# octree-nn/octfusion

Measured on AMD Instinct MI355X. Metric: denoising-steps/sec (depth-8 octree, batch 8), higher is better.
Workload: dtype f32 storage, fp16x3 products (fp16 hi + lo operand pairs = 22 significand bits, three fp16 MFMAs per product, fp32 accumulate)

## Files before the change

### include/ofx.h

```cpp
#ifndef OFX_H_
#define OFX_H_

#include <stddef.h>
#include <stdint.h>

#ifdef __cplusplus
extern "C" {
#endif

#define OFX_OK 0
#define OFX_EINVAL (-1)
#define OFX_ELAUNCH (-2)
#define OFX_ENODEV (-3)

#define OFX_ACT_NONE 0
#define OFX_ACT_SILU 1
#define OFX_ACT_GELU 2

#define OFX_MAX_DEPTH 16

int ofx_version(void);
const char* ofx_status_string(int status);
int ofx_device_check(void);
const char* ofx_build_hash(void);
// ... 140 lines not shown
int ofx_get_precision(void);
int64_t ofx_packed_floats(int64_t Kp, int64_t N);
int64_t ofx_packed_k(int64_t K);
int64_t ofx_graphconv_packed_k(int cin, int nt);
int ofx_pack_weights(const float* W, int64_t sk, int64_t sn, int64_t K, int64_t N,
                     int cin, int nt, float* Wp, int64_t Kp, void* stream);

int ofx_gemm_f32(const float* A, int64_t lda, const int32_t* a_rows, int64_t M, int64_t K,
                 const float* Wp, int64_t Kp, int64_t N, const float* bias,
                 const float* res, int64_t ldr, float* out, int64_t ldc,
                 const int32_t* out_rows, void* ws, size_t ws_bytes, void* stream);
int ofx_gemm_f32_planes(const float* A, int64_t lda, const int32_t* a_rows, int64_t M, int64_t K,
                        const float* Wp, int64_t Kp, int64_t N, const float* bias,
                        const float* res, int64_t ldr, float* out, int64_t ldc,
                        const int32_t* out_rows, void* ws, size_t ws_bytes, int out_mode, void* stream);

int ofx_graphconv_fwd(const float* x, int64_t ldx, int cin, int64_t n_nodes,
                      const int32_t* nbr, const int32_t* seg_ptr, const int32_t* col,
                      const int32_t* nbr_ext, const int32_t* multi_seg, int64_t n_multi, float* aux,
                      const float* type_frac, int64_t ldt, int nt_pad,
                      const float* Wp, int64_t Kp, int cout, const float* bias,
                      const float* emb, int64_t lde, const int32_t* batch_id,
                      const float* res, int64_t ldr, float* out, int64_t ldc,
                      double* stats , int64_t stats_ld,
                      void* ws, size_t ws_bytes, void* stream);

int ofx_graphconv_narrow_in(const float* x, int64_t ldx, int cin, int64_t n_nodes, const int32_t* seg_ptr,
                            const int32_t* col, const uint8_t* node_type, int nt, const float* W, int cout,
                            const float* bias, const int32_t* batch_id, float* out, int64_t ldc,
                            double* stats , int64_t stats_ld, void* ws, size_t ws_bytes, void* stream);
// ... 47 lines not shown
int ofx_graphconv_fwd_planes(const void* xp, int64_t ldx_bytes, int cin, int64_t n_nodes, const int32_t* seg_ptr,
                             const int32_t* col, const int32_t* nbr_ext, const int32_t* multi_seg, int64_t n_multi,
                             void* aux, size_t aux_bytes, const void* tfp, int64_t ldt_bytes, int nt, const void* W2,
                             int cout, const float* bias, const float* emb, int64_t lde, const int32_t* batch_id,
                             const float* res, int64_t ldr, float* out, int64_t ldc, double* stats ,
                             int64_t stats_ld, void* ws, size_t ws_bytes, void* sync , size_t sync_bytes,
                             int mode, int aux_ready, void* stream);
int ofx_graphconv_fwd_planes_cus(const void* xp, int64_t ldx_bytes, int cin, int64_t n_nodes, const int32_t* seg_ptr,
                                 const int32_t* col, const int32_t* nbr_ext, const int32_t* multi_seg, int64_t n_multi,
                                 void* aux, size_t aux_bytes, const void* tfp, int64_t ldt_bytes, int nt,
                                 const void* W2, int cout, const float* bias, const float* emb, int64_t lde,
                                 const int32_t* batch_id, const float* res, int64_t ldr, float* out, int64_t ldc,
                                 double* stats , int64_t stats_ld, void* ws, size_t ws_bytes,
                                 void* sync , size_t sync_bytes, int mode, int aux_ready, int cus,
                                 void* stream);
int ofx_set_gconv_persistent(int on);
int64_t ofx_gemm_planes_packed_bytes(int K, int N, int mode);
int ofx_pack_gemm_planes(const float* W, int64_t sk, int64_t sn, int K, int N, int mode, void* out, void* stream);
int ofx_gemm_planes(const void* ap, int64_t lda_bytes, int64_t n_a, int64_t M, int K, const int32_t* row_tab,
                    const void* W2, int N, const float* bias, float* out, int64_t ldc, int out_mode, void* ws,
                    size_t ws_bytes, void* sync, size_t sync_bytes, int mode, void* stream);
int ofx_set_gconv_cus(int cus);
int ofx_gconv3_plan(int64_t n_rows, int cout, int nkt, int wm, int ni, int cus, int32_t* out, int64_t out_len);
int ofx_set_gconv2_tile(int wm);

int ofx_grid_conv_table(int mode, int depth_out, int batch_size, int32_t pad, int32_t* nbr27,
                        void* stream);
int64_t ofx_conv3d_packed_k(int cin);
int ofx_pack_conv3d(const float* W, int cin, int cout, float* Wp, void* stream);
int ofx_gridconv_fwd(const float* x, int64_t ldx, int cin, int64_t n_in, int64_t n_out,
                     const int32_t* nbr27 ,
                     const int32_t* nbr27_ext ,
                     const float* zero_row ,
                     const float* Wp, int cout, const float* bias, const float* emb, int64_t lde,
                     const int32_t* batch_id, const float* res, int64_t ldr, float* out,
                     int64_t ldc, void* ws, size_t ws_bytes, void* stream);
int ofx_gather_gemm_f32(const float* x, int64_t ldx, int cin, int ntap, int64_t n_src, int64_t n_out, const int32_t* tab,
                        const float* zero_row, const float* Wp, int64_t Kp, int cout, const float* bias,
// ... 188 lines not shown
```

### octfusion_amd/_lib.py

```python
import ctypes
import os

import torch

_HERE = os.path.dirname(os.path.abspath(__file__))
LIB_PATH = os.environ.get('OFX_LIB', os.path.join(_HERE, 'libofx.so'))

c_p = ctypes.c_void_p
c_i = ctypes.c_int
c_l = ctypes.c_int64
c_f = ctypes.c_float
c_d = ctypes.c_double
c_sz = ctypes.c_size_t
c_u64 = ctypes.c_uint64


class OfxTree(ctypes.Structure):
    _fields_ = [('depth', c_i), ('full_depth', c_i), ('batch_size', c_i),
                ('child_all', c_p), ('key_all', c_p), ('leafrank_all', c_p),
                ('nnum_host', c_p), ('nnum_nempty_host', c_p)]


class OfxAdamRow(ctypes.Structure):
    _fields_ = [('param', c_p), ('grad', c_p), ('exp_avg', c_p), ('exp_avg_sq', c_p), ('ema', c_p), ('n', c_l)]
# ... 89 lines not shown
    'ofx_planes_split': (c_i, [c_p, c_l, c_l, c_i, c_i, c_i, c_p, c_l, c_p], True),
    'ofx_planes_merge': (c_i, [c_p, c_l, c_l, c_i, c_i, c_p, c_l, c_p], True),
    'ofx_gn_apply_planes': (c_i, [c_p, c_l, c_l, c_i, c_p, c_p, c_p, c_p, c_p, c_i, c_f, c_f, c_p, c_p, c_i, c_i, c_p,
                                  c_l, c_p, c_p, c_p, c_l, c_p, c_p, c_l, c_p], True),
    'ofx_gn_apply_planes_oct': (c_i, [c_p, c_l, c_l, c_i, c_p, c_p, c_p, c_p, c_p, c_i, c_f, c_f, c_p, c_p, c_i, c_i, c_p,
                                      c_l, c_l, c_p, c_p, c_p, c_l, c_i, c_p, c_p, c_l, c_p], True),
    'ofx_planes_packed_ktiles': (c_l, [c_i, c_i, c_i], False),
    'ofx_planes_packed_bytes': (c_l, [c_i, c_i, c_i, c_i], False),
    'ofx_pack_weights_planes': (c_i, [c_p, c_l, c_l, c_i, c_i, c_i, c_i, c_p, c_p], True),
    'ofx_graphconv_fwd_planes': (c_i, [c_p, c_l, c_i, c_l, c_p, c_p, c_p, c_p, c_l, c_p, c_sz, c_p, c_l, c_i, c_p, c_i,
                                       c_p, c_p, c_l, c_p, c_p, c_l, c_p, c_l, c_p, c_l, c_p, c_sz, c_p, c_sz, c_i, c_i,
                                       c_p], True),
    'ofx_graphconv_fwd_planes_cus': (c_i, [c_p, c_l, c_i, c_l, c_p, c_p, c_p, c_p, c_l, c_p, c_sz, c_p, c_l, c_i, c_p,
                                           c_i, c_p, c_p, c_l, c_p, c_p, c_l, c_p, c_l, c_p, c_l, c_p, c_sz, c_p, c_sz,
                                           c_i, c_i, c_i, c_p], True),
    'ofx_gn_finalize_window': (c_i, [c_p, c_p, c_i, c_i, c_i, c_i, c_i, c_f, c_f, c_p, c_p, c_p], True),
    'ofx_gn_apply_planes_window': (c_i, [c_p, c_l, c_l, c_i, c_i, c_i, c_p, c_p, c_p, c_p, c_p, c_i, c_f, c_f, c_p, c_p,
                                         c_i, c_i, c_p, c_l, c_p, c_p, c_p, c_l, c_p, c_p, c_l, c_p], True),
    'ofx_gn_apply_planes_oct_window': (c_i, [c_p, c_l, c_l, c_i, c_i, c_i, c_p, c_p, c_p, c_p, c_p, c_i, c_f, c_f, c_p,
                                             c_p, c_i, c_i, c_p, c_l, c_l, c_p, c_p, c_p, c_l, c_i, c_p, c_p, c_l, c_p],
                                       True),
    'ofx_set_gconv_persistent': (c_i, [c_i], True),
    'ofx_set_gconv_cus': (c_i, [c_i], True),
    'ofx_gemm_planes_packed_bytes': (c_l, [c_i, c_i, c_i], False),
    'ofx_pack_gemm_planes': (c_i, [c_p, c_l, c_l, c_i, c_i, c_i, c_p, c_p], True),
    'ofx_gemm_planes': (c_i, [c_p, c_l, c_l, c_l, c_i, c_p, c_p, c_i, c_p, c_p, c_l, c_i, c_p, c_sz, c_p, c_sz, c_i, c_p], False),
    'ofx_gconv3_plan': (c_i, [c_l, c_i, c_i, c_i, c_i, c_i, c_p, c_l], False),
    'ofx_set_gconv2_tile': (c_i, [c_i], True),
    'ofx_graph_multi_flag': (c_i, [c_p, c_l, c_p, c_p], True),
    'ofx_graph_primary_ext': (c_i, [c_p, c_p, c_l, c_p, c_p, c_p, c_p], True),
# ... 192 lines not shown
```

### octfusion_amd/csrc/ofx_gemm.hip

```cpp
#include "ofx_gemm_common.h"

constexpr int BM = 128;
constexpr int BK = 32;
constexpr int A_LD = BK + 4;
constexpr int MODE_DENSE = 0;
constexpr int MODE_GATHER = 1;

struct TileCoords { int split, tm, tn; };
__device__ __forceinline__ TileCoords tile_coords(const GemmArgs& g) {
  const int ntile = g.ntm * g.ntn;
  int bid = ofx_xcd_swizzle(blockIdx.x, ntile * g.nsplit);
  const int split = bid / ntile;
  bid -= split * ntile;
  const int tm = bid / g.ntn;
  return {split, tm, bid - tm * g.ntn};
}

__device__ __forceinline__ void load_a_dense(const GemmArgs& g, int64_t m0, int64_t k0, float4 (&va)[4]) {
  const int c4 = threadIdx.x & 7, r0 = threadIdx.x >> 3;
  const int64_t k = k0 + c4 * 4;
  const bool vec = ((g.lda & 3) == 0) && (k + 3 < g.K) && ((((uintptr_t)g.A) & 15) == 0);
#pragma unroll
  for (int i = 0; i < 4; ++i) {
    const int64_t m = m0 + r0 + 32 * i;
// ... 794 lines not shown
      }
      s += (double)v[i].x; q += (double)v[i].y;
    }
    if (sb >= 0) flush(sb, s, q);
  }
}

int ofx_launch_stats_reduce(const GemmArgs& g, int wr_rows, hipStream_t st) {
  const int64_t nwr = ofx_cdiv(g.M, wr_rows);
  stats_reduce_kernel<<<dim3((unsigned)ofx_cdiv(nwr, 64), (unsigned)ofx_cdiv(g.N, 64)), 256, 0, st>>>(
      g.stats_part, nwr, wr_rows, g.N, g.bid, g.stats, g.stats_ld);
  OFX_LAUNCH_CHECK();
  return OFX_OK;
}

template <int MODE>
static int launch_gemm(GemmArgs& g, float* ws, size_t ws_bytes, hipStream_t st) {
  if (g.M <= 0 || g.N <= 0) return OFX_OK;
  if (MODE == MODE_GATHER && !(g.fast && g.nbr_ext && g.aux && (!g.out_rows || g.gather_out_rows))) return OFX_EINVAL;
  {
    auto al16 = [](const void* p) { return (reinterpret_cast<uintptr_t>(p) & 15) == 0; };
    g.vec4 = g.N % 4 == 0 && al16(g.out) && g.ldc % 4 == 0 && (!g.res || (al16(g.res) && g.ldr % 4 == 0)) &&
             (!g.emb || (al16(g.emb) && g.lde % 4 == 0)) && (!g.bias || al16(g.bias));
  }
  const int bn = g.N <= 32 ? 32 : (g.N <= 64 ? 64 : 128);
  g.ntm = (int)ofx_cdiv(g.M, BM);
  g.ntn = (int)ofx_cdiv(g.N, bn);
  const int nkt = (int)(g.Kp / BK);
  int nsplit = 1;
  const int tiles = g.ntm * g.ntn;
  if (ws && tiles < 256 && nkt >= 8) {
    nsplit = (int)ofx_cdiv(512, tiles);
    if (nsplit > nkt / 4) nsplit = nkt / 4;
    if (nsplit > 64) nsplit = 64;
    const size_t per = (size_t)g.M * g.N * sizeof(float);
    if ((size_t)nsplit * per > ws_bytes) nsplit = (int)(ws_bytes / per);
    if (nsplit < 2) nsplit = 1;
  }
  g.kt_per_split = (int)ofx_cdiv(nkt, nsplit);
  nsplit = (int)ofx_cdiv(nkt, g.kt_per_split);
  g.nsplit = nsplit;
  g.ws = ws;
  bool fast = true;
  if (MODE == MODE_DENSE) {
    fast = ((g.lda & 3) == 0) && ((g.K & 3) == 0) && g.K >= 4 && ((((uintptr_t)g.A) & 15) == 0);
    if (fast) { g.ndir = 1; g.n_src = 0; g.aux = g.A; g.tf = g.A; g.ldt = g.lda; g.nbr_ext = (const int32_t*)g.A; }
  }
// ... 696 lines not shown
```

### octfusion_amd/csrc/ofx_gemm2.hip

```cpp
#include "ofx_planes.h"

template <int PREC, int WM, int NI>
__global__ void __launch_bounds__(512, 2) gconv2_kernel(const Gemm2Args a) {
  typedef G2Half<PREC, NI> Half;
  typedef G2Cfg<WM, NI> CF;
  constexpr int G2_NI = NI, G2_BN = CF::BN, G2_EPI_LOADS = CF::EPI_LOADS, RH = CF::READS;
  constexpr int G2_WM = WM, G2_BM = CF::BM, G2_A_BYTES = CF::A_BYTES, G2_BUF = CF::BUF, G2_TAB = CF::TAB;
  constexpr int G2_GLDS_PER_STEP = CF::GLDS;
  extern __shared__ __attribute__((aligned(128))) char smem2[];
  const GemmArgs& g = a.e;

  float osc = *g.oscale_p;
  asm volatile("" : "+s"(osc));
  const int ntile = g.ntm * g.ntn;
  const int bid = ofx_xcd_swizzle(blockIdx.x, ntile);
  const int tm = bid / g.ntn, tn = bid - tm * g.ntn;
  const int64_t m0 = a.row0 + (int64_t)tm * G2_BM, n0 = (int64_t)tn * G2_BN;

  const int lane = threadIdx.x & 63;
  const int wid = __builtin_amdgcn_readfirstlane(threadIdx.x >> 6);
  const int wm = wid >> 1, wn = wid & 1;
  const int l31 = lane & 31, h = lane >> 5;
  if (WM == 2 && a.stagger > 0 && blockIdx.x >= 256 && (int)blockIdx.x < a.prefetch) {
    const int grp = (int)blockIdx.x >> 8, ngrp = a.prefetch >> 8;
// ... 532 lines not shown
constexpr int G2_STAGGER_PER_KTILE = 1100;
extern "C" int ofx_set_gconv2_tile(int wm) {
  if (wm != 0 && wm != 2 && wm != 4) return OFX_EINVAL;
  g2_wm = wm;
  return OFX_OK;
}

static int g3_wm_pref = 0;
static int g3_auto_wm(int64_t M, int cout, int nkt, int ni) {
  (void)cout; (void)ni;
  if (g3_wm_pref == 2 || g3_wm_pref == 4) return g3_wm_pref;
  const int64_t U4 = ofx_cdiv(M, 256) * ofx_cdiv(cout, 64 * ni) * nkt;
  return U4 >= 3500 ? 4 : 2;
}
int ofx_launch_gconv3(Gemm2Args& a, int mode, int wm, int ni, void* ws_tail, size_t ws_tail_bytes, void* sync,
                      size_t sync_bytes, hipStream_t st, int nd = 7, int cus = 0);
static int g2_persistent = 1;
void ofx_gconv3_set_hybrid(int on);
extern "C" int ofx_set_gconv_persistent(int on) {
  if (on < 0 || on > 2) return OFX_EINVAL;
  g2_persistent = on ? 1 : 0;
  ofx_gconv3_set_hybrid(on == 2 ? 0 : 1);
  return OFX_OK;
}

extern "C" int ofx_graphconv_fwd_planes_cus(const void* xp, int64_t ldx_bytes, int cin, int64_t n_nodes,
                                            const int32_t* seg_ptr, const int32_t* col, const int32_t* nbr_ext,
                                            const int32_t* multi_seg, int64_t n_multi, void* aux, size_t aux_bytes,
                                            const void* tfp, int64_t ldt_bytes, int nt, const void* W2, int cout,
                                            const float* bias, const float* emb, int64_t lde, const int32_t* batch_id,
                                            const float* res, int64_t ldr, float* out, int64_t ldc, double* stats,
                                            int64_t stats_ld, void* ws, size_t ws_bytes, void* sync, size_t sync_bytes,
                                            int mode, int aux_ready, int cus, void* stream) {
  if (mode < 1 || mode > 3 || cus < 0 || (cus > 0 && cus < 8)) return OFX_EINVAL;
  const int64_t ch = g2_chunk(mode);
  if (n_nodes == 0 && cin >= 1 && cout >= 1) return OFX_OK;
  if (n_nodes < 0 || cin < 1 || (cin % ch) || cout < 1 || !xp || !seg_ptr || !col || !nbr_ext || !aux || !W2 || !out ||
      ldx_bytes < (int64_t)cin * (g2_pairs(mode) ? 4 : 2) || (ldx_bytes & 127) || ((uintptr_t)xp & 127) ||
      ((uintptr_t)aux & 127) || ((uintptr_t)W2 & 127) || ldc < cout || (res && ldr < cout) ||
      (emb && (!batch_id || lde < cout)) || n_multi < 0 || (n_multi > 0 && !multi_seg) || nt < 0)
    return OFX_EINVAL;
  if (aux_bytes < (size_t)(n_multi + 1) * (size_t)ldx_bytes) return OFX_EINVAL;
  const int ntc = nt > 1 ? nt : 0;
  if (ntc > 0 && (!tfp || (ldt_bytes & 127) || ((uintptr_t)tfp & 127) ||
                  ldt_bytes < (7 * (int64_t)ntc + ch - 1) / ch * G2_LINE))
    return OFX_EINVAL;
  if (stats && (!batch_id || stats_ld < cout)) return OFX_EINVAL;
  hipStream_t st = ofx_stream(stream);
  if (!aux_ready)
// ... 30 lines not shown
    a.row0 = row0;
    g.ntm = (int)ofx_cdiv(rows, wm * 64);
    a.stagger = wm == 2 ? G2_STAGGER_PER_KTILE * a.nkt : 0;
    a.prefetch = wm == 4 ? 256 : (ni == 1 ? 768 : 512);
    return mode == 2 ? G2_GO(2, wm) : (mode == 3 ? G2_GO(3, wm) : G2_GO(1, wm));
  };
  const int64_t tiles4 = ofx_cdiv(g.M, 256) * g.ntn;
  const int64_t tail4 = tiles4 % 256;
  const bool small_tail = tail4 > 0 && tail4 <= 64 && tiles4 < 1536;
  int wm_auto = (cout <= 128 && tiles4 < 2048) ? 2 : 4;
  if (cout > 128 && small_tail) wm_auto = 2;
  rc = 1;
  if (g2_persistent && sync) {
    size_t used = 0;
    if (g.stats_part) used = ((size_t)ofx_cdiv(g.M, 64) * (size_t)g.N * 2 * sizeof(float) + 255) & ~(size_t)255;
    const int wm3 = (g2_wm == 2 || g2_wm == 4) ? g2_wm : g3_auto_wm(g.M, cout, a.nkt, ni);
    if (ws && used <= ws_bytes)
      rc = ofx_launch_gconv3(a, mode, wm3, ni, (char*)ws + used, ws_bytes - used, sync, sync_bytes, st, 7, cus);
    if (rc < 0) return rc;
  }
  if (rc == 1) rc = launch((g2_wm == 2 || g2_wm == 4) ? g2_wm : wm_auto, 0, g.M);
#undef G2_GO
  if (rc) return rc;
  if (g.stats_part) {
    rc = ofx_launch_stats_reduce(g, 64, st);
    if (rc) return rc;
  }
  OFX_LAUNCH_CHECK();
  return OFX_OK;
}

extern "C" int ofx_graphconv_fwd_planes(const void* xp, int64_t ldx_bytes, int cin, int64_t n_nodes,
                                        const int32_t* seg_ptr, const int32_t* col, const int32_t* nbr_ext,
                                        const int32_t* multi_seg, int64_t n_multi, void* aux, size_t aux_bytes,
                                        const void* tfp, int64_t ldt_bytes, int nt, const void* W2, int cout,
                                        const float* bias, const float* emb, int64_t lde, const int32_t* batch_id,
                                        const float* res, int64_t ldr, float* out, int64_t ldc, double* stats,
                                        int64_t stats_ld, void* ws, size_t ws_bytes, void* sync, size_t sync_bytes,
                                        int mode, int aux_ready, void* stream) {
  return ofx_graphconv_fwd_planes_cus(xp, ldx_bytes, cin, n_nodes, seg_ptr, col, nbr_ext, multi_seg, n_multi, aux,
                                      aux_bytes, tfp, ldt_bytes, nt, W2, cout, bias, emb, lde, batch_id, res, ldr, out,
                                      ldc, stats, stats_ld, ws, ws_bytes, sync, sync_bytes, mode, aux_ready, 0, stream);
}

// ... 27 lines not shown
```

### octfusion_amd/csrc/ofx_gemm3.hip

```cpp
#include "ofx_planes.h"

constexpr int G3_NSP = 5;
constexpr int G3_KMIN = G3_NSP + 3;

template <int WM, int NI> struct G3Cfg : G2Cfg<WM, NI> {
  typedef G2Cfg<WM, NI> B;
  static constexpr int TAB = B::NBUF * B::BUF;
  static constexpr int RAW = TAB + B::BM * 32;
  static constexpr int RAW_WAVE = 32 * 28;
  static constexpr int LDS = RAW + B::BM * 28 + 128;
};

struct Gemm3Args {
  Gemm2Args b;
  int G;
  unsigned q, rem;
  unsigned U;
  int dp_rounds;
  float* part;
  unsigned* flags;
  unsigned* err;
  const char* nbr_lim;
  int snap;
  int early;
// ... 601 lines not shown
  if (hipGetDevice(&dev) != hipSuccess || dev < 0 || dev >= OFX_MAX_DEVICES) return 0;
  if (!cus[dev]) {
    int n = 0;
    if (hipDeviceGetAttribute(&n, hipDeviceAttributeMultiprocessorCount, dev) != hipSuccess) return 0;
    cus[dev] = n;
  }
  return cus[dev];
}
static int g3_cus() {
  const int n = g3_device_cus();
  return g3_cus_override > 0 && g3_cus_override < n ? g3_cus_override : n;
}

struct G3Plan { int G; unsigned q, rem, U; int dp_rounds; size_t part_bytes; };
static int g3_hybrid = 1;
static bool g3_plan(int64_t M, int cout, int nkt, int wm, int ni, G3Plan& p, int cus = 0) {
  if (cus <= 0) cus = g3_cus();
  if (cus < 8 || nkt < G3_KMIN) return false;
  const int64_t tiles = ofx_cdiv(M, wm * 64) * ofx_cdiv(cout, 64 * ni);
  if (tiles * nkt >= (1ll << 31)) return false;
  int64_t slots = ((int64_t)cus * (wm == 4 ? 1 : 2)) & ~7ll;
  int64_t G, region_tiles;
  int rounds = 0;
  if (tiles >= slots) {
    G = slots;
    rounds = g3_hybrid ? (int)(tiles / G - 1) : 0;
    region_tiles = tiles - (int64_t)rounds * G;
  } else {
    const int64_t U = tiles * nkt;
    G = slots < U / (2 * G3_KMIN) ? slots : U / (2 * G3_KMIN);
    G &= ~7ll;
    region_tiles = tiles;
  }
  if (G < 8) return false;
  const int64_t U = region_tiles * nkt;
  p.G = (int)G; p.U = (unsigned)U; p.q = (unsigned)(U / G); p.rem = (unsigned)(U % G); p.dp_rounds = rounds;
  p.part_bytes = (size_t)G * (size_t)(wm * 64) * (size_t)(64 * ni) * sizeof(float);
  return true;
}

void ofx_gconv3_set_hybrid(int on) { g3_hybrid = on ? 1 : 0; }
extern "C" int ofx_set_gconv_cus(int cus) {
  if (cus < 0 || (cus > 0 && cus < 8)) return OFX_EINVAL;
  g3_cus_override = cus;
  return OFX_OK;
}

extern "C" int ofx_gconv3_plan(int64_t n_rows, int cout, int nkt, int wm, int ni, int cus, int32_t* out, int64_t out_len) {
  G3Plan p;
  if (n_rows <= 0 || cout <= 0 || nkt <= 0 || (wm != 2 && wm != 4) || (ni != 1 && ni != 2)) return 0;
  if (!g3_plan(n_rows, cout, nkt, wm, ni, p, cus)) return 0;
  if (out) {
    if (out_len < 5 + (int64_t)p.G + 1) return 0;
    out[0] = p.G; out[1] = (int32_t)p.q; out[2] = (int32_t)p.rem; out[3] = (int32_t)p.U; out[4] = p.dp_rounds;
    for (int b = 0; b <= p.G; ++b) out[5 + b] = (int32_t)g3_bound((unsigned)b, p.q, p.rem, (unsigned)nkt, true);
  }
  return p.G;
}

int ofx_launch_gconv3(Gemm2Args& a, int mode, int wm, int ni, void* ws_tail, size_t ws_tail_bytes, void* sync,
                      size_t sync_bytes, hipStream_t st, int nd, int cus) {
  G3Plan p;
  GemmArgs& g = a.e;
  if (cus > 0) {
    const int dev_cus = g3_device_cus();
    if (dev_cus <= 0) return 1;
    if (cus > dev_cus) cus = dev_cus;
  }
  if (!sync || ((uintptr_t)sync & 3) || !ws_tail || ((uintptr_t)ws_tail & 15)) return 1;
  if (!g.vec4) return 1;
  if (!g3_plan(g.M, (int)g.N, a.nkt, wm, ni, p, cus)) return 1;
  if (p.part_bytes > ws_tail_bytes || (size_t)(p.G + 1) * sizeof(unsigned) > sync_bytes) return 1;
  if ((a.ldx >> 7) >= (1 << 20) || (a.ldt >> 7) >= (1 << 20) || a.n_src >= (1ll << 31)) return 1;
  Gemm3Args A = {};
  a.row0 = 0;
  g.ntm = (int)ofx_cdiv(g.M, wm * 64);
  A.b = a;
  A.G = p.G; A.q = p.q; A.rem = p.rem; A.U = p.U; A.dp_rounds = p.dp_rounds;
  A.part = (float*)ws_tail; A.flags = (unsigned*)sync;
  A.err = (unsigned*)sync + (sync_bytes / sizeof(unsigned) - 1);
  A.snap = 1;
  A.xcd_contig = 0;
  A.rt = p.U / (unsigned)a.nkt;
  A.early = p.q >= (unsigned)a.nkt ? 1 : 0;
  A.nbr_lim = (const char*)a.nbr_ext + ((((size_t)g.M * 28 - 4) >> 4) << 4);
  if (((uintptr_t)a.nbr_ext & 15)) return 1;
// ... 14 lines not shown
```

### octfusion_amd/graph_unet_hr.py

```python
import inspect

import torch
import torch.nn as nn

from . import ops
from .modules import (GraphConv, GraphDownsample, GraphResBlockEmbed, GraphUpsample, _Linear,
                      graphnormalization, skip_window)


def level_plan(input_depth, channel_mult, num_res_blocks):
    enc, dec = [], []
    d = input_depth
    last = len(channel_mult) - 1
    for level in range(len(channel_mult)):
        enc += [('res', d, level)] * num_res_blocks[level]
        if level != last:
            enc.append(('down', d, level))
            d -= 1
    for level in range(last, -1, -1):
        for i in range(num_res_blocks[level] + 1):
            dec.append(('res', d, level))
            if level and i == num_res_blocks[level]:
                dec.append(('up', d, level))
                d += 1
# ... 164 lines not shown

        if unet_lr is not None:
            c_mid = self.middle_block1.out_channels
            mid = torch.empty(n_at[d], 2 * c_mid, dtype=torch.float32, device=dev)
            h = self.middle_block1(h, emb, doctree, d, emb_act=emb_act, out=mid[:, :c_mid], emb_out=emb_outs[id(self.middle_block1)])
            ahead_ok = ops.SKIP_AHEAD and not ops.LANE_CUS and not isinstance(unet_lr, UNet3DModel)
            ahead_main, ahead_side = ops.skip_ahead_stream(dev) if ahead_ok else (None, None)
            if ahead_side is not None:
                todo, si = [], len(hs)
                for (kind, dd, _), module in zip(self._dec, self.output_blocks):
                    if kind == 'res':
                        si -= 1
                        win = skip_window(self._cat_plan[si][0], self._cat_plan[si][1], module.block1_norm.group)
                        if win is not None:
                            todo.append((n_at[dd] * (win[1] - win[0]) * module.out_channels, si, dd, module))
                with torch.cuda.stream(ahead_side):
                    for _, si, dd, module in sorted(todo, key=lambda t_: -t_[0]):
                        module.prepare_skip(cat_bufs[si], doctree, dd, ops.SKIP_AHEAD_CUS, c_h=self._cat_plan[si][0],
                                            skip_stats=ops.get_stats(hs[si]))
            if 'out' in inspect.signature(unet_lr.forward_as_middle).parameters:
                h_lr = unet_lr.forward_as_middle(h, doctree, timesteps, label, context, out=mid[:, c_mid:])
            else:
                h_lr = unet_lr.forward_as_middle(h, doctree, timesteps, label, context)
            if h_lr.data_ptr() == mid[:, c_mid:].data_ptr() and h_lr.shape[1] == c_mid:
                h = ops.cat_channels(h, h_lr, buf=mid)
            else:
                h = ops.cat_channels(h, h_lr)
            if ahead_side is not None:
                ahead_main.wait_stream(ahead_side)
            last = len(cat_bufs) - 1
            h = self.middle_block2(h, emb, doctree, d, emb_act=emb_act, emb_out=emb_outs[id(self.middle_block2)],
                                   out=cat_bufs[last][:, :self._cat_plan[last][0]])

        n_skip = len(hs)
        j = 0
        pending = h
        for idx, ((kind, dd, _), module) in enumerate(zip(self._dec, self.output_blocks)):
            nxt_is_res = idx + 1 < len(self._dec) and self._dec[idx + 1][0] == 'res'
# ... 30 lines not shown
```

### octfusion_amd/modules.py

```python
import math

import torch
import torch.nn as nn

from . import ops


def _gn_groups(channels, group=32):
    if channels <= 32:
        group = channels // 4
    elif channels % group != 0:
        group = 30
    assert channels % group == 0
    return group


class GraphConv(nn.Module):

    def __init__(self, in_channels, out_channels, n_edge_type=7, avg_degree=7, n_node_type=0,
                 use_bias=False):
        super().__init__()
        assert n_edge_type == 7, 'the dual octree graph has 7 edge types'
        self.in_channels = in_channels
        self.out_channels = out_channels
# ... 379 lines not shown
        hit = self._pw2_win.get((part, mode, window))
        if hit is not None and hit[0] == key:
            return hit[1]
        c_lo, c_hi = window
        w3 = w.detach().view(7, conv.in_channels + nt, conv.out_channels)
        if part == 'early':
            ww, cin_w, nt_w = w3[:, c_lo:c_hi], c_hi - c_lo, 0
        else:
            ww, cin_w, nt_w = torch.cat([w3[:, :c_lo], w3[:, conv.in_channels:]], dim=1), c_lo, conv.n_node_type
        ww = ww.contiguous().view(-1, conv.out_channels)
        pw = ops.PackedPlanes().get(ww, cin_w, nt_w, mode)
        self._pw2_win[(part, mode, window)] = (key, pw)
        return pw

    @torch.no_grad()
    def prepare_skip(self, x_cat, doctree, depth, cus=0, c_h=None, skip_stats=None):
        self._ahead = None
        conv, norm = self.conv1, self.block1_norm
        C = self.channels
        mode = conv.planes_mode(doctree, depth)
        win = skip_window(c_h, C - c_h, norm.group) if c_h is not None and 0 < c_h < C else None
        if (win is None or skip_stats is None or not ops.planes_pairs(mode) or x_cat.shape[1] != C
                or (win[1] - win[0]) < ops.SKIP_AHEAD_MIN_SHARE * C):
            return False
        n, dev, B = x_cat.shape[0], x_cat.device, doctree.batch_size
        seg_ptr, col, _, _ = doctree.csr(depth)
        _, multi_seg, n_multi = doctree.ext(depth)
        oct_plan = doctree.oct_plan(depth) if ops.AUX_PLAN == 'oct' else None
        block_plan = doctree.aux_plan(depth) if ops.AUX_PLAN and oct_plan is None else None
        g = ops.AuxGraph(seg_ptr, col, multi_seg, n_multi, oct_plan, block_plan)
        hp = torch.empty(n, C, dtype=torch.float32, device=dev)
        if not ops.planes_ok(hp, mode):
            return False
        aux = torch.empty((n_multi + 2) * C * 4, dtype=torch.uint8, device=dev)
        sums = torch.empty(B, C, 2, dtype=torch.float64, device=dev)
        sums[:, c_h:].copy_(skip_stats.view(B, C - c_h, 2))
        mean = rstd = None
        if ops._gn_launch(mode, g, n * C, C // norm.group)[1]:
            mean = torch.empty(B * C, dtype=torch.float32, device=dev)
            rstd = torch.empty(B * C, dtype=torch.float32, device=dev)
        ops.group_norm_window(x_cat, doctree.batch_id32(depth), doctree.count(depth), B, norm.weights, norm.bias,
                              norm.group, win, sums.view(-1), hp, aux, mode, g, norm.eps, 'silu', mean, rstd)
        part = ops.graphconv_planes(hp, mode, seg_ptr, col, doctree.ext(depth), self._window_pack('early', mode, win),
                                    win[1] - win[0], 0, window=win, cus=cus)
        self._ahead = dict(buf=x_cat.data_ptr(), c_h=c_h, win=win, mode=mode, g=g, hp=hp, aux=aux, sums=sums, mean=mean,
                           rstd=rstd, part=part, depth=depth)
        return True

    def ahead_pending(self, x_cat, h_stats=None):
        a = self._ahead
        if a is None or a['buf'] != x_cat.data_ptr():
            return False
        a['h_stats'] = h_stats
        return True

    def _finish_ahead(self, x, doctree, depth, emb_out):
        a, self._ahead = self._ahead, None
        conv, norm = self.conv1, self.block1_norm
        c_h, (c_lo, c_hi), mode, B = a['c_h'], a['win'], a['mode'], doctree.batch_size
# ... 96 lines not shown
```

### octfusion_amd/ops.py

```python
import contextlib
import os
from typing import NamedTuple

import torch

from . import _lib
from ._lib import call, call_may_decline, ptr, stream

ACT = {None: 0, 'none': 0, 'silu': 1, 'gelu': 2}

GRAPHCONV_PROFILE = None
_NO_BRACKET = contextlib.nullcontext()


@contextlib.contextmanager
def _timed_layer(prof, *rec):
    e0 = torch.cuda.Event(enable_timing=True)
    e1 = torch.cuda.Event(enable_timing=True)
    e0.record()
    yield
    e1.record()
    prof.append((e0, e1) + rec)


# ... 194 lines not shown
            wp = torch.zeros(7, cin_pad + ntc, N, dtype=torch.float32, device=w.device)
            w3 = w.view(7, cin + ntc, N)
            wp[:, :cin] = w3[:, :cin]
            wp[:, cin_pad:] = w3[:, cin:]
            w = wp.view(7 * (cin_pad + ntc), N)
            cin, K = cin_pad, 7 * (cin_pad + ntc)
        L = _lib.lib()
        out = torch.empty(L.ofx_planes_packed_bytes(cin, nt, N, mode), dtype=torch.uint8, device=w.device)
        call('ofx_pack_weights_planes', ptr(w), N, 1, cin, nt, N, mode, ptr(out), stream())
        self.t, self.key, self.N, self.K, self.cin, self.nt = out, key, N, k_logical, cin_logical, nt
        self.nkt = L.ofx_planes_packed_ktiles(cin, nt, mode)
        return self


def graphconv_planes(xp, mode, seg_ptr, col, ext, pw, cin, nt, tf_planes=None, bias=None, emb=None, batch_id=None,
                     res=None, out=None, stats=None, window=None, cus=0):
    assert planes_of(xp) == mode
    N = xp.shape[0]
    bpc = 4 if planes_pairs(mode) else 2
    ldx = xp.stride(0) * bpc if N > 1 else xp.shape[1] * bpc
    c_lo = 0
    if window is not None:
        c_lo, c_hi = window
        assert planes_pairs(mode) and c_lo % 32 == 0 and c_hi % 32 == 0 and 0 <= c_lo < c_hi <= xp.shape[1]
        assert cin == c_hi - c_lo
    else:
        assert xp.shape[1] == cin
    off = c_lo * bpc
    out, ldc = _out2d(out, N, pw.N, xp.device)
    nbr_ext, multi_seg, n_multi = ext
    aux = getattr(xp, AUX_ATTR, None)
# ... 9 lines not shown
    ldt = tf_planes.stride(0) * bpc if tf_planes is not None else 0
    _chk(bias)
    _chk(stats, torch.float64)
    E = col.numel()
    flops = 2.0 * N * pw.K * pw.N
    nbytes = bpc * (E * pw.cin + pw.K * pw.N) + 4.0 * N * pw.N + 8.0 * E
    with _layer_bracket(flops, nbytes, pw.N, ('graph2' if planes_pairs(mode) else 'graph2h', N, pw.cin, pw.N)):
        ws = workspace(xp.device)
        sync = sync_words(xp.device)
        _meta('graphconv', flops, 0, (N, pw.cin, pw.N, 'planes', 'emb' if emb is not None else '',
                                      'res' if res is not None else '', 'stats' if stats is not None else ''))
        args = (ptr(xp) + off, ldx, cin, N, ptr(seg_ptr), ptr(col), ptr(nbr_ext), ptr(multi_seg), n_multi, ptr(aux) + off,
                aux.numel() * aux.element_size() - off, ptr(tf_planes), ldt, nt, ptr(pw.t), pw.N, ptr(bias), ptr(emb), lde,
                ptr(batch_id) if (emb is not None or stats is not None) else None, ptr(res), ldr, ptr(out), ldc,
                ptr(stats), pw.N, ptr(ws), ws.numel(), ptr(sync), sync.numel() * 4, mode, aux_ready)
        if cus:
            call('ofx_graphconv_fwd_planes_cus', *args, int(cus), stream())
        else:
            call('ofx_graphconv_fwd_planes', *args, stream())
    return out


SKIP_AHEAD = os.environ.get('OFX_SKIP_AHEAD', '1') == '1'
SKIP_AHEAD_CUS = int(os.environ.get('OFX_SKIP_AHEAD_CUS', '128'))
SKIP_AHEAD_MIN_SHARE = float(os.environ.get('OFX_SKIP_AHEAD_MIN_SHARE', '0'))


def skip_ahead_stream(device):
    if device.type != 'cuda':
        return None, None
    s = _scratch('skip_ahead', device, False, lambda: torch.cuda.Stream(device))
    main = torch.cuda.current_stream(device)
    if main.cuda_stream == s.cuda_stream:
        return None, None
    s.wait_stream(main)
    return main, s


SIDE_STREAM = os.environ.get('OFX_SIDE_STREAM', '0') == '1'

# ... 904 lines not shown
```

Before: 123.6.

## Partition CUs between skip-ahead side stream and main GEMMs, reorder skip prep

Adds per-launch plan control (CU count, warp tile, blocks per CU) for the persistent graph-conv kernel on the skip-ahead side stream. Adds a global GEMM CU budget that changes the split-K decision, used to cap the main-stream low-res middle GEMMs at a CU share while side work runs. Reverses the skip-prep order when the level is large. The aim is better concurrency between the side-stream skip convs and the main-stream middle UNet. The risk is that split-K GEMMs become less parallel when the global budget is reduced.

Result: no change. 124.5 (median of 6 runs) (+0.8%).

```diff
diff --git a/include/ofx.h b/include/ofx.h
--- a/include/ofx.h
+++ b/include/ofx.h
@@ -178,6 +178,8 @@
                         const float* Wp, int64_t Kp, int64_t N, const float* bias,
                         const float* res, int64_t ldr, float* out, int64_t ldc,
                         const int32_t* out_rows, void* ws, size_t ws_bytes, int out_mode, void* stream);
+int ofx_set_gemm_cus(int cus);
+int ofx_get_gemm_cus(void);
 
 int ofx_graphconv_fwd(const float* x, int64_t ldx, int cin, int64_t n_nodes,
                       const int32_t* nbr, const int32_t* seg_ptr, const int32_t* col,
@@ -255,6 +257,14 @@
                                  double* stats , int64_t stats_ld, void* ws, size_t ws_bytes,
                                  void* sync , size_t sync_bytes, int mode, int aux_ready, int cus,
                                  void* stream);
+int ofx_graphconv_fwd_planes_plan(const void* xp, int64_t ldx_bytes, int cin, int64_t n_nodes, const int32_t* seg_ptr,
+                                  const int32_t* col, const int32_t* nbr_ext, const int32_t* multi_seg, int64_t n_multi,
+                                  void* aux, size_t aux_bytes, const void* tfp, int64_t ldt_bytes, int nt,
+                                  const void* W2, int cout, const float* bias, const float* emb, int64_t lde,
+                                  const int32_t* batch_id, const float* res, int64_t ldr, float* out, int64_t ldc,
+                                  double* stats , int64_t stats_ld, void* ws, size_t ws_bytes,
+                                  void* sync , size_t sync_bytes, int mode, int aux_ready, int cus, int wm,
+                                  int blocks_per_cu, void* stream);
 int ofx_set_gconv_persistent(int on);
 int64_t ofx_gemm_planes_packed_bytes(int K, int N, int mode);
 int ofx_pack_gemm_planes(const float* W, int64_t sk, int64_t sn, int K, int N, int mode, void* out, void* stream);
@@ -263,6 +273,8 @@
                     size_t ws_bytes, void* sync, size_t sync_bytes, int mode, void* stream);
 int ofx_set_gconv_cus(int cus);
 int ofx_gconv3_plan(int64_t n_rows, int cout, int nkt, int wm, int ni, int cus, int32_t* out, int64_t out_len);
+int ofx_gconv3_plan2(int64_t n_rows, int cout, int nkt, int wm, int ni, int cus, int blocks_per_cu, int32_t* out,
+                     int64_t out_len);
 int ofx_set_gconv2_tile(int wm);
 
 int ofx_grid_conv_table(int mode, int depth_out, int batch_size, int32_t pad, int32_t* nbr27,
diff --git a/octfusion_amd/_lib.py b/octfusion_amd/_lib.py
--- a/octfusion_amd/_lib.py
+++ b/octfusion_amd/_lib.py
@@ -127,6 +127,12 @@
     'ofx_graphconv_fwd_planes_cus': (c_i, [c_p, c_l, c_i, c_l, c_p, c_p, c_p, c_p, c_l, c_p, c_sz, c_p, c_l, c_i, c_p,
                                            c_i, c_p, c_p, c_l, c_p, c_p, c_l, c_p, c_l, c_p, c_l, c_p, c_sz, c_p, c_sz,
                                            c_i, c_i, c_i, c_p], True),
+    'ofx_graphconv_fwd_planes_plan': (c_i, [c_p, c_l, c_i, c_l, c_p, c_p, c_p, c_p, c_l, c_p, c_sz, c_p, c_l, c_i, c_p,
+                                            c_i, c_p, c_p, c_l, c_p, c_p, c_l, c_p, c_l, c_p, c_l, c_p, c_sz, c_p, c_sz,
+                                            c_i, c_i, c_i, c_i, c_i, c_p], True),
+    'ofx_gconv3_plan2': (c_i, [c_l, c_i, c_i, c_i, c_i, c_i, c_i, c_p, c_l], False),
+    'ofx_set_gemm_cus': (c_i, [c_i], True),
+    'ofx_get_gemm_cus': (c_i, [], False),
     'ofx_gn_finalize_window': (c_i, [c_p, c_p, c_i, c_i, c_i, c_i, c_i, c_f, c_f, c_p, c_p, c_p], True),
     'ofx_gn_apply_planes_window': (c_i, [c_p, c_l, c_l, c_i, c_i, c_i, c_p, c_p, c_p, c_p, c_p, c_i, c_f, c_f, c_p, c_p,
                                          c_i, c_i, c_p, c_l, c_p, c_p, c_p, c_l, c_p, c_p, c_l, c_p], True),
diff --git a/octfusion_amd/csrc/ofx_gemm.hip b/octfusion_amd/csrc/ofx_gemm.hip
--- a/octfusion_amd/csrc/ofx_gemm.hip
+++ b/octfusion_amd/csrc/ofx_gemm.hip
@@ -832,6 +832,14 @@
   return OFX_OK;
 }
 
+static int g_gemm_cus = 0;
+extern "C" int ofx_set_gemm_cus(int cus) {
+  if (cus < 0 || (cus > 0 && cus < 8)) return OFX_EINVAL;
+  g_gemm_cus = cus;
+  return OFX_OK;
+}
+extern "C" int ofx_get_gemm_cus() { return g_gemm_cus; }
+
 template <int MODE>
 static int launch_gemm(GemmArgs& g, float* ws, size_t ws_bytes, hipStream_t st) {
   if (g.M <= 0 || g.N <= 0) return OFX_OK;
@@ -847,8 +855,9 @@
   const int nkt = (int)(g.Kp / BK);
   int nsplit = 1;
   const int tiles = g.ntm * g.ntn;
-  if (ws && tiles < 256 && nkt >= 8) {
-    nsplit = (int)ofx_cdiv(512, tiles);
+  const int cus = g_gemm_cus > 0 ? g_gemm_cus : 256;
+  if (ws && tiles < cus && nkt >= 8) {
+    nsplit = (int)ofx_cdiv(2 * cus, tiles);
     if (nsplit > nkt / 4) nsplit = nkt / 4;
     if (nsplit > 64) nsplit = 64;
     const size_t per = (size_t)g.M * g.N * sizeof(float);
diff --git a/octfusion_amd/csrc/ofx_gemm2.hip b/octfusion_amd/csrc/ofx_gemm2.hip
--- a/octfusion_amd/csrc/ofx_gemm2.hip
+++ b/octfusion_amd/csrc/ofx_gemm2.hip
@@ -570,7 +570,8 @@
   return U4 >= 3500 ? 4 : 2;
 }
 int ofx_launch_gconv3(Gemm2Args& a, int mode, int wm, int ni, void* ws_tail, size_t ws_tail_bytes, void* sync,
-                      size_t sync_bytes, hipStream_t st, int nd = 7, int cus = 0);
+                      size_t sync_bytes, hipStream_t st, int nd = 7, int cus = 0, int bpc = 0);
+int ofx_gconv3_plan_bpc(int64_t n_rows, int cout, int nkt, int wm, int ni, int cus, int bpc, int32_t* out, int64_t out_len);
 static int g2_persistent = 1;
 void ofx_gconv3_set_hybrid(int on);
 extern "C" int ofx_set_gconv_persistent(int on) {
@@ -580,15 +581,26 @@
   return OFX_OK;
 }
 
-extern "C" int ofx_graphconv_fwd_planes_cus(const void* xp, int64_t ldx_bytes, int cin, int64_t n_nodes,
-                                            const int32_t* seg_ptr, const int32_t* col, const int32_t* nbr_ext,
-                                            const int32_t* multi_seg, int64_t n_multi, void* aux, size_t aux_bytes,
-                                            const void* tfp, int64_t ldt_bytes, int nt, const void* W2, int cout,
-                                            const float* bias, const float* emb, int64_t lde, const int32_t* batch_id,
-                                            const float* res, int64_t ldr, float* out, int64_t ldc, double* stats,
-                                            int64_t stats_ld, void* ws, size_t ws_bytes, void* sync, size_t sync_bytes,
-                                            int mode, int aux_ready, int cus, void* stream) {
+extern "C" int ofx_gconv3_plan2(int64_t n_rows, int cout, int nkt, int wm, int ni, int cus, int blocks_per_cu,
+                                int32_t* out, int64_t out_len) {
+  if ((wm != 0 && wm != 2 && wm != 4) || blocks_per_cu < 0 || blocks_per_cu > 2 || (blocks_per_cu == 2 && wm != 2) ||
+      n_rows <= 0 || cout <= 0 || nkt <= 0 || (ni != 1 && ni != 2))
+    return 0;
+  if (wm == 0) wm = (g2_wm == 2 || g2_wm == 4) ? g2_wm : g3_auto_wm(n_rows, cout, nkt, ni);
+  return ofx_gconv3_plan_bpc(n_rows, cout, nkt, wm, ni, cus, blocks_per_cu, out, out_len);
+}
+
+extern "C" int ofx_graphconv_fwd_planes_plan(const void* xp, int64_t ldx_bytes, int cin, int64_t n_nodes,
+                                             const int32_t* seg_ptr, const int32_t* col, const int32_t* nbr_ext,
+                                             const int32_t* multi_seg, int64_t n_multi, void* aux, size_t aux_bytes,
+                                             const void* tfp, int64_t ldt_bytes, int nt, const void* W2, int cout,
+                                             const float* bias, const float* emb, int64_t lde, const int32_t* batch_id,
+                                             const float* res, int64_t ldr, float* out, int64_t ldc, double* stats,
+                                             int64_t stats_ld, void* ws, size_t ws_bytes, void* sync, size_t sync_bytes,
+                                             int mode, int aux_ready, int cus, int wm, int blocks_per_cu, void* stream) {
   if (mode < 1 || mode > 3 || cus < 0 || (cus > 0 && cus < 8)) return OFX_EINVAL;
+  if ((wm != 0 && wm != 2 && wm != 4) || blocks_per_cu < 0 || blocks_per_cu > 2 || (blocks_per_cu == 2 && wm != 2))
+    return OFX_EINVAL;
   const int64_t ch = g2_chunk(mode);
   if (n_nodes == 0 && cin >= 1 && cout >= 1) return OFX_OK;
   if (n_nodes < 0 || cin < 1 || (cin % ch) || cout < 1 || !xp || !seg_ptr || !col || !nbr_ext || !aux || !W2 || !out ||
@@ -649,9 +661,10 @@
   if (g2_persistent && sync) {
     size_t used = 0;
     if (g.stats_part) used = ((size_t)ofx_cdiv(g.M, 64) * (size_t)g.N * 2 * sizeof(float) + 255) & ~(size_t)255;
-    const int wm3 = (g2_wm == 2 || g2_wm == 4) ? g2_wm : g3_auto_wm(g.M, cout, a.nkt, ni);
+    const int wm3 = wm ? wm : ((g2_wm == 2 || g2_wm == 4) ? g2_wm : g3_auto_wm(g.M, cout, a.nkt, ni));
     if (ws && used <= ws_bytes)
-      rc = ofx_launch_gconv3(a, mode, wm3, ni, (char*)ws + used, ws_bytes - used, sync, sync_bytes, st, 7, cus);
+      rc = ofx_launch_gconv3(a, mode, wm3, ni, (char*)ws + used, ws_bytes - used, sync, sync_bytes, st, 7, cus,
+                             blocks_per_cu);
     if (rc < 0) return rc;
   }
   if (rc == 1) rc = launch((g2_wm == 2 || g2_wm == 4) ? g2_wm : wm_auto, 0, g.M);
@@ -663,6 +676,20 @@
   }
   OFX_LAUNCH_CHECK();
   return OFX_OK;
+}
+
+extern "C" int ofx_graphconv_fwd_planes_cus(const void* xp, int64_t ldx_bytes, int cin, int64_t n_nodes,
+                                            const int32_t* seg_ptr, const int32_t* col, const int32_t* nbr_ext,
+                                            const int32_t* multi_seg, int64_t n_multi, void* aux, size_t aux_bytes,
+                                            const void* tfp, int64_t ldt_bytes, int nt, const void* W2, int cout,
+                                            const float* bias, const float* emb, int64_t lde, const int32_t* batch_id,
+                                            const float* res, int64_t ldr, float* out, int64_t ldc, double* stats,
+                                            int64_t stats_ld, void* ws, size_t ws_bytes, void* sync, size_t sync_bytes,
+                                            int mode, int aux_ready, int cus, void* stream) {
+  return ofx_graphconv_fwd_planes_plan(xp, ldx_bytes, cin, n_nodes, seg_ptr, col, nbr_ext, multi_seg, n_multi, aux,
+                                       aux_bytes, tfp, ldt_bytes, nt, W2, cout, bias, emb, lde, batch_id, res, ldr, out,
+                                       ldc, stats, stats_ld, ws, ws_bytes, sync, sync_bytes, mode, aux_ready, cus, 0, 0,
+                                       stream);
 }
 
 extern "C" int ofx_graphconv_fwd_planes(const void* xp, int64_t ldx_bytes, int cin, int64_t n_nodes,
diff --git a/octfusion_amd/csrc/ofx_gemm3.hip b/octfusion_amd/csrc/ofx_gemm3.hip
--- a/octfusion_amd/csrc/ofx_gemm3.hip
+++ b/octfusion_amd/csrc/ofx_gemm3.hip
@@ -639,12 +639,14 @@
 
 struct G3Plan { int G; unsigned q, rem, U; int dp_rounds; size_t part_bytes; };
 static int g3_hybrid = 1;
-static bool g3_plan(int64_t M, int cout, int nkt, int wm, int ni, G3Plan& p, int cus = 0) {
+static bool g3_plan(int64_t M, int cout, int nkt, int wm, int ni, G3Plan& p, int cus = 0, int bpc = 0) {
   if (cus <= 0) cus = g3_cus();
   if (cus < 8 || nkt < G3_KMIN) return false;
+  const int fit = wm == 4 ? 1 : 2;
+  if (bpc < 0 || bpc > fit) return false;
   const int64_t tiles = ofx_cdiv(M, wm * 64) * ofx_cdiv(cout, 64 * ni);
   if (tiles * nkt >= (1ll << 31)) return false;
-  int64_t slots = ((int64_t)cus * (wm == 4 ? 1 : 2)) & ~7ll;
+  int64_t slots = ((int64_t)cus * (bpc ? bpc : fit)) & ~7ll;
   int64_t G, region_tiles;
   int rounds = 0;
   if (tiles >= slots) {
@@ -671,10 +673,10 @@
   return OFX_OK;
 }
 
-extern "C" int ofx_gconv3_plan(int64_t n_rows, int cout, int nkt, int wm, int ni, int cus, int32_t* out, int64_t out_len) {
+int ofx_gconv3_plan_bpc(int64_t n_rows, int cout, int nkt, int wm, int ni, int cus, int bpc, int32_t* out, int64_t out_len) {
   G3Plan p;
   if (n_rows <= 0 || cout <= 0 || nkt <= 0 || (wm != 2 && wm != 4) || (ni != 1 && ni != 2)) return 0;
-  if (!g3_plan(n_rows, cout, nkt, wm, ni, p, cus)) return 0;
+  if (!g3_plan(n_rows, cout, nkt, wm, ni, p, cus, bpc)) return 0;
   if (out) {
     if (out_len < 5 + (int64_t)p.G + 1) return 0;
     out[0] = p.G; out[1] = (int32_t)p.q; out[2] = (int32_t)p.rem; out[3] = (int32_t)p.U; out[4] = p.dp_rounds;
@@ -682,9 +684,12 @@
   }
   return p.G;
 }
+extern "C" int ofx_gconv3_plan(int64_t n_rows, int cout, int nkt, int wm, int ni, int cus, int32_t* out, int64_t out_len) {
+  return ofx_gconv3_plan_bpc(n_rows, cout, nkt, wm, ni, cus, 0, out, out_len);
+}
 
 int ofx_launch_gconv3(Gemm2Args& a, int mode, int wm, int ni, void* ws_tail, size_t ws_tail_bytes, void* sync,
-                      size_t sync_bytes, hipStream_t st, int nd, int cus) {
+                      size_t sync_bytes, hipStream_t st, int nd, int cus, int bpc) {
   G3Plan p;
   GemmArgs& g = a.e;
   if (cus > 0) {
@@ -694,7 +699,7 @@
   }
   if (!sync || ((uintptr_t)sync & 3) || !ws_tail || ((uintptr_t)ws_tail & 15)) return 1;
   if (!g.vec4) return 1;
-  if (!g3_plan(g.M, (int)g.N, a.nkt, wm, ni, p, cus)) return 1;
+  if (!g3_plan(g.M, (int)g.N, a.nkt, wm, ni, p, cus, bpc)) return 1;
   if (p.part_bytes > ws_tail_bytes || (size_t)(p.G + 1) * sizeof(unsigned) > sync_bytes) return 1;
   if ((a.ldx >> 7) >= (1 << 20) || (a.ldt >> 7) >= (1 << 20) || a.n_src >= (1ll << 31)) return 1;
   Gemm3Args A = {};
diff --git a/octfusion_amd/graph_unet_hr.py b/octfusion_amd/graph_unet_hr.py
--- a/octfusion_amd/graph_unet_hr.py
+++ b/octfusion_amd/graph_unet_hr.py
@@ -1,3 +1,4 @@
+import contextlib
 import inspect
 
 import torch
@@ -202,14 +203,18 @@
                         win = skip_window(self._cat_plan[si][0], self._cat_plan[si][1], module.block1_norm.group)
                         if win is not None:
                             todo.append((n_at[dd] * (win[1] - win[0]) * module.out_channels, si, dd, module))
+                shadow = bool(todo) and max(n_at[t_[2]] for t_ in todo) >= ops.SKIP_AHEAD_SHADOW_MIN_ROWS
+                todo.sort(key=lambda t_: -t_[0], reverse=shadow and ops.SKIP_AHEAD_REVERSE)
                 with torch.cuda.stream(ahead_side):
-                    for _, si, dd, module in sorted(todo, key=lambda t_: -t_[0]):
-                        module.prepare_skip(cat_bufs[si], doctree, dd, ops.SKIP_AHEAD_CUS, c_h=self._cat_plan[si][0],
-                                            skip_stats=ops.get_stats(hs[si]))
-            if 'out' in inspect.signature(unet_lr.forward_as_middle).parameters:
-                h_lr = unet_lr.forward_as_middle(h, doctree, timesteps, label, context, out=mid[:, c_mid:])
-            else:
-                h_lr = unet_lr.forward_as_middle(h, doctree, timesteps, label, context)
+                    for k, (_, si, dd, module) in enumerate(todo):
+                        module.prepare_skip(cat_bufs[si], doctree, dd, c_h=self._cat_plan[si][0],
+                                            skip_stats=ops.get_stats(hs[si]), plan=ops.skip_ahead_plan(k))
+            share = ops.SKIP_AHEAD_GEMM_CUS if ahead_side is not None and shadow else 0
+            with (ops.gemm_cus(share) if share else contextlib.nullcontext()):
+                if 'out' in inspect.signature(unet_lr.forward_as_middle).parameters:
+                    h_lr = unet_lr.forward_as_middle(h, doctree, timesteps, label, context, out=mid[:, c_mid:])
+                else:
+                    h_lr = unet_lr.forward_as_middle(h, doctree, timesteps, label, context)
             if h_lr.data_ptr() == mid[:, c_mid:].data_ptr() and h_lr.shape[1] == c_mid:
                 h = ops.cat_channels(h, h_lr, buf=mid)
             else:
diff --git a/octfusion_amd/modules.py b/octfusion_amd/modules.py
--- a/octfusion_amd/modules.py
+++ b/octfusion_amd/modules.py
@@ -417,7 +417,7 @@
         return pw
 
     @torch.no_grad()
-    def prepare_skip(self, x_cat, doctree, depth, cus=0, c_h=None, skip_stats=None):
+    def prepare_skip(self, x_cat, doctree, depth, cus=0, c_h=None, skip_stats=None, plan=None):
         self._ahead = None
         conv, norm = self.conv1, self.block1_norm
         C = self.channels
@@ -445,7 +445,7 @@
         ops.group_norm_window(x_cat, doctree.batch_id32(depth), doctree.count(depth), B, norm.weights, norm.bias,
                               norm.group, win, sums.view(-1), hp, aux, mode, g, norm.eps, 'silu', mean, rstd)
         part = ops.graphconv_planes(hp, mode, seg_ptr, col, doctree.ext(depth), self._window_pack('early', mode, win),
-                                    win[1] - win[0], 0, window=win, cus=cus)
+                                    win[1] - win[0], 0, window=win, cus=cus, plan=plan)
         self._ahead = dict(buf=x_cat.data_ptr(), c_h=c_h, win=win, mode=mode, g=g, hp=hp, aux=aux, sums=sums, mean=mean,
                            rstd=rstd, part=part, depth=depth)
         return True
diff --git a/octfusion_amd/ops.py b/octfusion_amd/ops.py
--- a/octfusion_amd/ops.py
+++ b/octfusion_amd/ops.py
@@ -232,7 +232,7 @@
 
 
 def graphconv_planes(xp, mode, seg_ptr, col, ext, pw, cin, nt, tf_planes=None, bias=None, emb=None, batch_id=None,
-                     res=None, out=None, stats=None, window=None, cus=0):
+                     res=None, out=None, stats=None, window=None, cus=0, plan=None):
     assert planes_of(xp) == mode
     N = xp.shape[0]
     bpc = 4 if planes_pairs(mode) else 2
@@ -272,7 +272,9 @@
                 aux.numel() * aux.element_size() - off, ptr(tf_planes), ldt, nt, ptr(pw.t), pw.N, ptr(bias), ptr(emb), lde,
                 ptr(batch_id) if (emb is not None or stats is not None) else None, ptr(res), ldr, ptr(out), ldc,
                 ptr(stats), pw.N, ptr(ws), ws.numel(), ptr(sync), sync.numel() * 4, mode, aux_ready)
-        if cus:
+        if plan is not None:
+            call('ofx_graphconv_fwd_planes_plan', *args, int(plan[0]), int(plan[1]), int(plan[2]), stream())
+        elif cus:
             call('ofx_graphconv_fwd_planes_cus', *args, int(cus), stream())
         else:
             call('ofx_graphconv_fwd_planes', *args, stream())
@@ -282,6 +284,36 @@
 SKIP_AHEAD = os.environ.get('OFX_SKIP_AHEAD', '1') == '1'
 SKIP_AHEAD_CUS = int(os.environ.get('OFX_SKIP_AHEAD_CUS', '128'))
 SKIP_AHEAD_MIN_SHARE = float(os.environ.get('OFX_SKIP_AHEAD_MIN_SHARE', '0'))
+
+
+def _skip_ahead_plan(text, cus):
+    plan = [tuple(int(v) for v in t.split(':')) for t in text.replace(',', ' ').split()]
+    if not plan:
+        return [(cus, 0, 0)] * 5
+    for p in plan:
+        if len(p) != 3 or p[1] not in (0, 2, 4) or p[2] not in (0, 1, 2) or (p[2] == 2 and p[1] != 2) or 0 < p[0] < 8 or p[0] < 0:
+            raise ValueError('OFX_SKIP_AHEAD_PLAN: bad triple %r (cus:wm:blocks_per_cu)' % (p,))
+    return plan
+
+
+SKIP_AHEAD_PLAN = _skip_ahead_plan(os.environ.get('OFX_SKIP_AHEAD_PLAN', ''), SKIP_AHEAD_CUS)
+SKIP_AHEAD_REVERSE = os.environ.get('OFX_SKIP_AHEAD_REVERSE', '1') == '1'
+SKIP_AHEAD_GEMM_CUS = int(os.environ.get('OFX_SKIP_AHEAD_GEMM_CUS', '128'))
+SKIP_AHEAD_SHADOW_MIN_ROWS = int(os.environ.get('OFX_SKIP_AHEAD_SHADOW_MIN_ROWS', '160000'))
+
+
+def skip_ahead_plan(i):
+    return SKIP_AHEAD_PLAN[min(i, len(SKIP_AHEAD_PLAN) - 1)]
+
+
+@contextlib.contextmanager
+def gemm_cus(cus):
+    prev = _lib.lib().ofx_get_gemm_cus()
+    call('ofx_set_gemm_cus', int(cus))
+    try:
+        yield
+    finally:
+        call('ofx_set_gemm_cus', prev)
 
 
 def skip_ahead_stream(device):
```
